# AlexGr5/StereoVision

Measured on AMD Instinct MI355X. Metric: disparity frames/sec + HBM GB/s, 1920x1080 D=128 win=9, 1/2/4/8 GPU, higher is better.
Workload: dtype u8

## Files before the change

### stereovision_amd/csrc/sv_match.hip

```cpp
#include "sv_internal.h"
#include "sv_xcd.h"

#include <algorithm>
#include <cstdlib>
#include <vector>
#include <cstdio>
#include <type_traits>

namespace sv {
namespace {

constexpr int COST_SAD4 = 4;

__host__ __device__ __forceinline__ int seg_width(int lpg, int dpl, int sm = 4) { return (sm * lpg + dpl - 1) / dpl * dpl; }
__host__ __device__ __forceinline__ int wave_cols(int lpg, int dpl, int sm = 4) { return (64 / lpg) * seg_width(lpg, dpl, sm); }
int seg_mult(int kind, int r) {
    static const int sm4 = [] {
        const char* e = std::getenv("SV_SAD4_SEG");
        const int v = e ? std::atoi(e) : 0;
        return v >= 1 && v <= 8 ? v : 0;
    }();
    if (kind != COST_SAD4) return 4;
    if (sm4) return sm4;
    return (2 * r - 2 + 3) / 4 <= 2 ? 4 : 2;
// ... 376 lines not shown
                    h[k][q] = __builtin_amdgcn_sad_hi_u8(L.w[NC + q], rn[sk].w[NC + q], h[k][q]) - m;
                }
                continue;
            }
            uint32_t vn[ROWS];
            ccol<COST, ND, NW>(L, rn[sk], vn);
            if constexpr (RUN) {
                uint32_t vo[ROWS];
                ccol<COST, ND, NW>(LO, ro[sk], vo);
#pragma unroll
                for (int q = 0; q < ROWS; ++q) h[k][q] = shl_add(vn[q] - vo[q], 1 << dbits, h[k][q]);
            } else {
                h[k][0] = (vn[0] << dbits) | mk[k];
            }
        }
#pragma unroll
        for (int q = 0; q < ROWS; ++q) {
            uint32_t b = 0xFFFFFFFFu;
#pragma unroll
            for (int k = 0; k < DPL; ++k) b = min(b, h[k][q]);
            bk[q][u] = b;
        }
        __builtin_amdgcn_sched_barrier(0);
    }
}

template <int LPG, int N>
__device__ __forceinline__ void reduce_batch(uint32_t* v) {
#define SV_ROR_STEP(CTRL)                                                                     \
    _Pragma("unroll") for (int i = 0; i < N; ++i)                                             \
        v[i] = min(v[i], (uint32_t)__builtin_amdgcn_update_dpp(0u, (int)v[i], CTRL, 0xF, 0xF, false));
    SV_ROR_STEP(0x121)
    SV_ROR_STEP(0x122)
    SV_ROR_STEP(0x124)
    SV_ROR_STEP(0x128)
#undef SV_ROR_STEP
    if constexpr (LPG >= 32) {
#pragma unroll
        for (int i = 0; i < N; ++i)
            v[i] = min(v[i], (uint32_t)__builtin_amdgcn_update_dpp(-1, (int)v[i], 0x142, 0xA, 0xF, false));
    }
    if constexpr (LPG == 64) {
#pragma unroll
        for (int i = 0; i < N; ++i)
            v[i] = min(v[i], (uint32_t)__builtin_amdgcn_update_dpp(-1, (int)v[i], 0x143, 0xC, 0xF, false));
    }
}

__device__ __forceinline__ void reduce_scatter16(uint32_t (&v)[16], int l) {
#define SV_RS_STEP(HALF, BIT, CTRL)                                                            \
    {                                                                                          \
        const bool hi = (l & (BIT)) != 0;                                                      \
        _Pragma("unroll") for (int k = 0; k < (HALF); ++k) {                                   \
            const uint32_t send = hi ? v[k] : v[k + (HALF)];                                   \
            const uint32_t keep = hi ? v[k + (HALF)] : v[k];                                   \
            v[k] = min(keep, (uint32_t)__builtin_amdgcn_update_dpp(0u, (int)send, CTRL, 0xF, 0xF, false)); \
        }                                                                                      \
    }
    SV_RS_STEP(8, 8, 0x140)
    SV_RS_STEP(4, 4, 0x141)
    SV_RS_STEP(2, 2, 0x1B)
    SV_RS_STEP(1, 1, 0xB1)
#undef SV_RS_STEP
}

__device__ __forceinline__ void reduce_scatter16_bm(uint32_t (&v)[16], int l) {
#define SV_BM_PAIR(A, B, CTRL, M0, M1)                                                          \
    "v_min_u32_dpp %" #A ", %" #A ", %" #A " " CTRL " row_mask:0xf bank_mask:" M0 "\n\t"      \
    "v_min_u32_dpp %" #A ", %" #B ", %" #B " " CTRL " row_mask:0xf bank_mask:" M1 "\n\t"
    asm volatile("s_nop 1\n\t"
                 SV_BM_PAIR(0, 8, "row_mirror", "0x3", "0xc") SV_BM_PAIR(1, 9, "row_mirror", "0x3", "0xc")
                 SV_BM_PAIR(2, 10, "row_mirror", "0x3", "0xc") SV_BM_PAIR(3, 11, "row_mirror", "0x3", "0xc")
                 SV_BM_PAIR(4, 12, "row_mirror", "0x3", "0xc") SV_BM_PAIR(5, 13, "row_mirror", "0x3", "0xc")
                 SV_BM_PAIR(6, 14, "row_mirror", "0x3", "0xc") SV_BM_PAIR(7, 15, "row_mirror", "0x3", "0xc")
                 : "+v"(v[0]), "+v"(v[1]), "+v"(v[2]), "+v"(v[3]), "+v"(v[4]), "+v"(v[5]), "+v"(v[6]), "+v"(v[7])
                 : "v"(v[8]), "v"(v[9]), "v"(v[10]), "v"(v[11]), "v"(v[12]), "v"(v[13]), "v"(v[14]), "v"(v[15]));
    asm volatile("s_nop 1\n\t"
                 SV_BM_PAIR(0, 4, "row_half_mirror", "0x5", "0xa") SV_BM_PAIR(1, 5, "row_half_mirror", "0x5", "0xa")
                 SV_BM_PAIR(2, 6, "row_half_mirror", "0x5", "0xa") SV_BM_PAIR(3, 7, "row_half_mirror", "0x5", "0xa")
                 : "+v"(v[0]), "+v"(v[1]), "+v"(v[2]), "+v"(v[3])
                 : "v"(v[4]), "v"(v[5]), "v"(v[6]), "v"(v[7]));
#undef SV_BM_PAIR
#define SV_RS_STEP(HALF, BIT, CTRL)                                                            \
    {                                                                                          \
        const bool hi = (l & (BIT)) != 0;                                                      \
        _Pragma("unroll") for (int k = 0; k < (HALF); ++k) {                                   \
            const uint32_t send = hi ? v[k] : v[k + (HALF)];                                   \
            const uint32_t keep = hi ? v[k + (HALF)] : v[k];                                   \
            v[k] = min(keep, (uint32_t)__builtin_amdgcn_update_dpp(0u, (int)send, CTRL, 0xF, 0xF, false)); \
        }                                                                                      \
    }
    SV_RS_STEP(2, 2, 0x1B)
    SV_RS_STEP(1, 1, 0xB1)
#undef SV_RS_STEP
}

__device__ __forceinline__ void reduce_scatter8_bm(uint32_t (&v)[8], int l) {
#define SV_BM_PAIR(A, B, CTRL, M0, M1)                                                          \
    "v_min_u32_dpp %" #A ", %" #A ", %" #A " " CTRL " row_mask:0xf bank_mask:" M0 "\n\t"      \
    "v_min_u32_dpp %" #A ", %" #B ", %" #B " " CTRL " row_mask:0xf bank_mask:" M1 "\n\t"
    asm volatile("s_nop 1\n\t"
                 SV_BM_PAIR(0, 4, "row_mirror", "0x3", "0xc") SV_BM_PAIR(1, 5, "row_mirror", "0x3", "0xc")
                 SV_BM_PAIR(2, 6, "row_mirror", "0x3", "0xc") SV_BM_PAIR(3, 7, "row_mirror", "0x3", "0xc")
                 : "+v"(v[0]), "+v"(v[1]), "+v"(v[2]), "+v"(v[3])
                 : "v"(v[4]), "v"(v[5]), "v"(v[6]), "v"(v[7]));
    asm volatile("s_nop 1\n\t"
                 SV_BM_PAIR(0, 2, "row_half_mirror", "0x5", "0xa") SV_BM_PAIR(1, 3, "row_half_mirror", "0x5", "0xa")
                 : "+v"(v[0]), "+v"(v[1])
                 : "v"(v[2]), "v"(v[3]));
#undef SV_BM_PAIR
    const bool hi = (l & 2) != 0;
    const uint32_t send = hi ? v[0] : v[1];
    const uint32_t keep = hi ? v[1] : v[0];
    v[0] = min(keep, (uint32_t)__builtin_amdgcn_update_dpp(0u, (int)send, 0x1B, 0xF, 0xF, false));
    v[0] = min(v[0], (uint32_t)__builtin_amdgcn_update_dpp(0u, (int)v[0], 0xB1, 0xF, 0xF, false));
}

template <int COST, int ND> struct Occ {
    static constexpr int W = COST == COST_SAD4 ? 2 : (COST == COST_SAD || ND <= 3) ? 3 : 2;
};

template <int COST, int ND, int DPL>
__global__ __launch_bounds__((64 * PackCfg<COST, ND>::WPB), (Occ<COST, ND>::W)) void k_match(MatchParams a) {
    constexpr int NW = PackCfg<COST, ND>::NW;
    constexpr int ROWS = PackCfg<COST, ND>::ROWS;
    extern __shared__ __attribute__((aligned(16))) uint4 smem[];
    if (blockIdx.z) {
        a.L += blockIdx.z * a.fs_in;
        a.R += blockIdx.z * a.fs_in;
        a.out += blockIdx.z * a.fs_out;
        if constexpr (COST == COST_HOG) {
            a.HL += blockIdx.z * a.fs_hist;
            a.HR += blockIdx.z * a.fs_hist;
        }
    }
    const int lane = threadIdx.x & 63;
    const int wid = PackCfg<COST, ND>::WPB == 1 ? 0 : (int)(threadIdx.x >> 6);
    const int LPG = a.lpg;
    const int S = seg_width(LPG, DPL, a.segm);
    const int WC = wave_cols(LPG, DPL, a.segm);
    const int r = a.r;
    const int W2 = 2 * r + 1;
    const int c0 = (DPL - (4 * r + 1) % DPL) % DPL;
    const int NL = WC + 4 * r + DPL + 1;
    const int NRlog = WC + 4 * r + LPG * DPL + DPL;
    const int NRphys = NRlog + (NRlog + c0) / DPL + 1;
    using P = PackCfg<COST, ND>;
    uint4* wbase = reinterpret_cast<uint4*>(reinterpret_cast<char*>(smem) + (size_t)wid * (NL + NRphys) * P::SLOT_BYTES);
    typename P::CT* cbase = reinterpret_cast<typename P::CT*>(wbase + (size_t)(NL + NRphys) * P::QX);
    const PackOut<COST, ND> Lw{wbase, cbase};
    const PackOut<COST, ND> Rw{wbase + (size_t)NL * P::QX, cbase + NL};
    const PackPtr<COST, ND> Lp{Lw.x, Lw.c};
    const PackPtr<COST, ND> Rp{Rw.x, Rw.c};

    const int y = a.row0 + ((int)blockIdx.y * PackCfg<COST, ND>::WPB + wid) * ROWS;
    const int yc = min(y, a.row1 - 1);
    const int xw = a.X0 + (int)blockIdx.x * WC;
    const int cL0 = xw - 3 * r - 1;
    const int cR0 = cL0 - a.minD - (LPG * DPL - 1);

    build_all_packs<COST, ND, DPL>(a, yc, cL0, NL, cR0, NRlog, c0, Lw, Rw, lane);

    if (blockIdx.x == 0) {
        const int16_t inv = (int16_t)((a.minD - 1) * 16);
#pragma unroll
        for (int q = 0; q < ROWS; ++q) {
            if (y + q >= a.row1) break;
            int16_t* orow = a.out + (size_t)(y + q) * a.opitch;
            for (int x = lane; x < a.X0; x += 64) orow[x] = inv;
            for (int x = a.X1 + lane; x < a.W; x += 64) orow[x] = inv;
        }
    }
    __syncthreads();
    if (y >= a.row1) return;

    const int g = lane >> a.lpg_log2;
    const int l = lane & (LPG - 1);
    const int sl = l ^ (((lane >> 4) & 1) << 3);
    const int xs = xw + g * S;
    const int iL0 = g * S + 2 * r + 1;
    const int iR0 = g * S + 2 * r + (LPG - sl) * DPL;
    const uint32_t dmask = (1u << a.dbits) - 1u;
    const int dbits = a.dbits;
    const int j = l - (LPG - 16);

    uint32_t mk[DPL];
    uint32_t h[DPL][ROWS], bk[ROWS][DPL];
#pragma unroll
    for (int k = 0; k < DPL; ++k) {
        const int idx = sl * DPL + k;
        mk[k] = idx < a.D ? (uint32_t)idx : 0xFFFFFFFFu;
#pragma unroll
        for (int q = 0; q < ROWS; ++q) h[k][q] = idx < a.D ? (uint32_t)idx : a.pad_key | (uint32_t)idx;
    }

    for (int t = 0; t < W2; ++t) {
        const Pk<NW> L = ld<COST, ND>(Lp + (iL0 + t));
#pragma unroll
        for (int k = 0; k < DPL; ++k) {
            uint32_t vn[ROWS];
            ccol<COST, ND, NW>(L, ld<COST, ND>(Rp + rslot(iR0 + t - k, c0, DPL)), vn);
            if constexpr (COST == COST_HOG) h[k][0] = (vn[0] << dbits) | mk[k];
            else {
#pragma unroll
                for (int q = 0; q < ROWS; ++q) h[k][q] += vn[q] << dbits;
            }
        }
    }
    {
        const bool emit0 = j == 0 && xs < a.X1;
#pragma unroll
        for (int q = 0; q < ROWS; ++q) {
            uint32_t b = 0xFFFFFFFFu;
#pragma unroll
            for (int k = 0; k < DPL; ++k) b = min(b, h[k][q]);
            if (LPG == 16) reduce_batch<16, 1>(&b);
            else if (LPG == 32) reduce_batch<32, 1>(&b);
            else reduce_batch<64, 1>(&b);
            if (emit0 && y + q < a.row1)
                a.out[(size_t)(y + q) * a.opitch + xs] = (int16_t)(((int)(b & dmask) + a.minD) * 16);
        }
    }

    const int phi = (DPL - W2 % DPL) % DPL;
    const int cut = DPL - phi;
    const int iN = iR0 + W2;
    Pk<NW> rn[DPL], ro[DPL];
#pragma unroll
    for (int s = 1; s < DPL; ++s) {
        rn[s] = ld<COST, ND>(Rp + rslot(iN - (DPL - s), c0, DPL));
        if constexpr (COST != COST_HOG) ro[s] = ld<COST, ND>(Rp + rslot(iR0 - (DPL - s), c0, DPL));
    }
    const PackPtr<COST, ND> rn0 = Rp + rslot(iN, c0, DPL);
    const PackPtr<COST, ND> ro0 = Rp + rslot(iR0, c0, DPL);
    const PackPtr<COST, ND> ln0 = Lp + (iL0 + W2);
    const PackPtr<COST, ND> lo0 = Lp + iL0;
    const int T = (S - 1 + DPL - 1) / DPL * DPL;

    for (int t0 = 0, c = 0; t0 < T; t0 += DPL, ++c) {
        match_chunk<COST, ND, DPL>(cut, dbits, rn0 + c * (DPL + 1), ro0 + c * (DPL + 1), ln0 + t0, lo0 + t0, rn,
                                   ro, h, mk, bk);
        if constexpr (ROWS * DPL == 16 || ROWS * DPL == 32) {
            if (LPG == 16) {
#pragma unroll
                for (int half = 0; half < ROWS * DPL / 16; ++half) {
                    uint32_t v[16];
#pragma unroll
                    for (int i = 0; i < 16; ++i) v[i] = bk[(16 * half + i) / DPL][i % DPL];
                    reduce_scatter16(v, l);
                    const int q = (16 * half) / DPL + l / DPL, e = t0 + l % DPL + 1, x = xs + e;
                    if (e < S && x < a.X1 && y + q < a.row1)
                        a.out[(size_t)(y + q) * a.opitch + x] = (int16_t)(((int)(v[0] & dmask) + a.minD) * 16);
                }
                continue;
            }
        }
        if constexpr (ROWS * DPL == 8) {
            uint32_t v[8];
#pragma unroll
            for (int i = 0; i < 8; ++i) v[i] = bk[i / DPL][i % DPL];
            reduce_scatter8_bm(v, lane & 15);
            uint32_t key = v[0];
            if (LPG >= 32) {
                const auto p = __builtin_amdgcn_permlane16_swap(key, key, false, false);
                key = min(p[0], p[1]);
            }
            if (LPG == 64) {
                const auto p = __builtin_amdgcn_permlane32_swap(key, key, false, false);
                key = min(p[0], p[1]);
            }
            const int i = (l >> 1) & 7, q = i / DPL, e = t0 + i % DPL + 1, x = xs + e;
            if (l < 16 && (l & 1) == 0 && e < S && x < a.X1 && y + q < a.row1)
                a.out[(size_t)(y + q) * a.opitch + x] = (int16_t)(((int)(key & dmask) + a.minD) * 16);
            continue;
        }
        const int e = t0 + j + 1;
        const int x = xs + e;
        const bool emit = j >= 0 && j < DPL && e < S && x < a.X1;
        if (LPG == 16) reduce_batch<16, ROWS * DPL>(&bk[0][0]);
        else if (LPG == 32) reduce_batch<32, ROWS * DPL>(&bk[0][0]);
        else reduce_batch<64, ROWS * DPL>(&bk[0][0]);
#pragma unroll
        for (int q = 0; q < ROWS; ++q) {
            uint32_t v = bk[q][0];
#pragma unroll
            for (int u = 1; u < DPL; ++u) v = (j == u) ? bk[q][u] : v;
            if (emit && y + q < a.row1)
                a.out[(size_t)(y + q) * a.opitch + x] = (int16_t)(((int)(v & dmask) + a.minD) * 16);
        }
    }
}

constexpr int RG_DPL = 4;

typedef unsigned short u16x2 __attribute__((ext_vector_type(2)));
__device__ __forceinline__ uint32_t pk_add16(uint32_t a, uint32_t b) {
    return __builtin_bit_cast(uint32_t, __builtin_bit_cast(u16x2, a) + __builtin_bit_cast(u16x2, b));
}
__device__ __forceinline__ uint32_t pk_sub16(uint32_t a, uint32_t b) {
    return __builtin_bit_cast(uint32_t, __builtin_bit_cast(u16x2, a) - __builtin_bit_cast(u16x2, b));
}


template <int R, int LPGT, bool DEFER, bool KEYS, bool SSD = false>
__global__ __launch_bounds__(64, 2) void k_match_ring(MatchParams a) {
    using P = PackCfg<COST_SAD4, R>;
    constexpr int NW = P::NW, NC = P::NC, W2 = 2 * R + 1;
    constexpr bool PK = R >= 6;
    static_assert(P::SPLIT && (P::CW == 3) == PK, "ring kind expects split packs (20 B for r 2..3, 24 B for r 4..5, 28 B for r 6..7)");
    extern __shared__ __attribute__((aligned(16))) uint4 smem[];
    int bx, by, bz;
    xcd_tile(a.xcd_map != 0, bx, by, bz);
    if (bz) {
        a.L += bz * a.fs_in;
        a.R += bz * a.fs_in;
        a.out += bz * a.fs_out;
        if constexpr (KEYS) a.keys += bz * a.fs_out;
    }
    const int lane = threadIdx.x;
    constexpr int LPG = LPGT;
    const int S = a.segm;
    const int WC = (64 / LPG) * S;
    constexpr bool SADU = PK || R <= 5;
    constexpr int M = SADU ? W2 + 1 : W2;
    constexpr int U = M % 4 == 0 ? M : M % 2 == 0 ? 2 * M : 4 * M;
    constexpr int NCH = U / 4;
    const int Tn = (S + 2 * R + 3) & ~3;
    const int nit = (Tn + U - 1) / U;
    const int e0 = (nit * U - Tn) >> 2;
    const int NL = WC - S + Tn + 1;
    const int NRlog = WC - S + Tn + 4 * LPG;
    constexpr int c0 = 1;
    const int NRphys = NRlog + (NRlog + c0) / RG_DPL + 1;
    uint4* wbase = smem;
    typename P::CT* cbase = reinterpret_cast<typename P::CT*>(wbase + (size_t)(NL + NRphys));
    const PackOut<COST_SAD4, R> Lw{wbase, cbase};
    const PackOut<COST_SAD4, R> Rw{wbase + NL, cbase + NL};
    const PackPtr<COST_SAD4, R> Lp{Lw.x, Lw.c};
    const PackPtr<COST_SAD4, R> Rp{Rw.x, Rw.c};

    const int y = a.row0 + by * 4;
    const int yc = min(y, a.row1 - 1);
    const int xw = a.X0 + bx * WC;
    const int cL0 = xw - R;
    const int cR0 = cL0 - a.minD - (4 * LPG - 1);
    build_ring_packs<R, 3, RG_DPL>(a, yc, cL0, NL, cR0, NRlog, c0, Lw, Rw, lane);

    if (!KEYS && bx == 0) {
        const int16_t inv = (int16_t)((a.minD - 1) * 16);
#pragma unroll
        for (int q = 0; q < 4; ++q) {
            if (y + q >= a.row1) break;
            int16_t* orow = a.out + (size_t)(y + q) * a.opitch;
            for (int x = lane; x < a.X0; x += 64) orow[x] = inv;
            for (int x = a.X1 + lane; x < a.W; x += 64) orow[x] = inv;
        }
    }
    __syncthreads();
    if (y >= a.row1) return;

    const int g = lane / LPG;
    const int l = lane & (LPG - 1);
    const int xs = xw + g * S;
    const int dl = PK ? min(4 * l, a.D - 4) : 4 * l;
    const int iR0 = g * S + 4 * (LPG - 1) - dl + 3;
    constexpr int RQ = PK ? 2 : 4;
    uint32_t h[RG_DPL][RQ], lab[RG_DPL];
#pragma unroll
    for (int k = 0; k < RG_DPL; ++k) {
        const int idx = 4 * l + k;
        const uint32_t base = PK ? 0u : idx < a.D ? (uint32_t)idx : (SSD ? a.pad_key : 0x8000u << 16) | (uint32_t)idx;
        lab[k] = (uint32_t)idx;
#pragma unroll
        for (int q = 0; q < RQ; ++q) h[k][q] = base;
    }
    uint32_t ring[M][RG_DPL][RQ];
#pragma unroll
    for (int s = 0; s < M; ++s)
#pragma unroll
        for (int k = 0; k < RG_DPL; ++k)
#pragma unroll
            for (int q = 0; q < RQ; ++q) ring[s][k][q] = 0u;
    Pk<NW> rn[RG_DPL];
#pragma unroll
    for (int s = 1; s < RG_DPL; ++s) rn[RG_DPL - s] = ld<COST_SAD4, R, true>(Rp + rslot(iR0 - s, c0, RG_DPL));
    PackPtr<COST_SAD4, R> rb = Rp + (rslot(iR0, c0, RG_DPL) - e0 * (RG_DPL + 1));
    PackPtr<COST_SAD4, R> lb = Lp + (g * S - 4 * e0);
    constexpr bool LPF = !(R == 5 && SADU);
    Pk<NW> Lnext = ld<COST_SAD4, R, true>(lb + 4 * e0);
    const int jq = (lane >> 2) & 3, ju = (lane >> 1) & 1;
    constexpr bool join2 = LPG >= 32;
    int pofs = 0;
    if (join2) {
        const auto p = __builtin_amdgcn_permlane16_swap((uint32_t)lane, (uint32_t)lane + 64u, false, false);
        pofs = (max(p[0], p[1]) < 64u) ? 0 : 2;
    }
    const int eb = ju - 2 * R + pofs;
    constexpr int OB = KEYS ? 4 : 2;
    const int ooff = OB * ((y + jq) * a.opitch + xs + eb);
    const auto orsrc = KEYS ? __builtin_amdgcn_make_buffer_rsrc(a.keys, 0, 0x7FFFFFFF, 0x00020000)
                            : __builtin_amdgcn_make_buffer_rsrc(a.out, 0, 0x7FFFFFFF, 0x00020000);
    const int emax = ((l & 1) == 0 && l < (join2 ? 32 : 16) && y + jq < a.row1) ? max(0, min(S, a.X1 - xs)) : 0;

    auto emit_key = [&](uint32_t key, int tt) {
        const int off = (unsigned)(tt + eb) < (unsigned)emax ? ooff + OB * tt : (int)0x80000000u;
        if constexpr (KEYS) __builtin_amdgcn_raw_buffer_store_b32(key, orsrc, off, 0, 0);
        else __builtin_amdgcn_raw_buffer_store_b16(
            (uint16_t)(((int)(key & (SSD ? (1u << a.dbits) - 1u : 0xFFFFu)) + a.minD) * 16), orsrc, off, 0, 0);
    };
    auto join_pairs = [&](uint32_t kA_, uint32_t kB_) {
        auto p = __builtin_amdgcn_permlane16_swap(kA_, kB_, false, false);
        uint32_t key = min(p[0], p[1]);
        if (LPG == 64) {
            p = __builtin_amdgcn_permlane32_swap(key, key, false, false);
            key = min(p[0], p[1]);
        }
        return key;
    };
    auto join_rows = [&](uint32_t key) {
        if (LPG >= 32) {
            const auto p = __builtin_amdgcn_permlane16_swap(key, key, false, false);
            key = min(p[0], p[1]);
        }
        if (LPG == 64) {
            const auto p = __builtin_amdgcn_permlane32_swap(key, key, false, false);
            key = min(p[0], p[1]);
        }
        return key;
    };
    uint32_t dv[8], kA = 0xFFFFFFFFu;
    int tprev = -(1 << 24);
#pragma unroll
    for (int i = 0; i < 8; ++i) dv[i] = 0xFFFFFFFFu;

    for (int it = 0, t0 = -4 * e0; it < nit; ++it) {
#pragma unroll
        for (int ch = 0; ch < NCH; ++ch, t0 += 4) {
            if (t0 < 0) continue;
            uint32_t bk[4][2];
#pragma unroll
            for (int u = 0; u < 4; ++u) {
                const int slot = (4 * ch + u) % M, oslot = (4 * ch + u + 1) % M;
                rn[u] = ld<COST_SAD4, R, true>(rb + (ch * (RG_DPL + 1) + u));
                const Pk<NW> Lc = LPF ? Lnext : ld<COST_SAD4, R, true>(lb + (4 * ch + u));
                if constexpr (LPF) Lnext = ld<COST_SAD4, R, true>(lb + (4 * ch + u + 1));
                uint32_t sqL[4];
                if constexpr (SSD) {
                    uint32_t sc = 0u;
#pragma unroll
                    for (int i = 0; i < NC; ++i) sc = __builtin_amdgcn_udot4(Lc.w[i], Lc.w[i], sc, false);
#pragma unroll
                    for (int q = 0; q < 4; ++q)
                        sqL[q] = __builtin_amdgcn_udot4(Lc.w[NC + q], Lc.w[NC + q], sc, false) << a.dbits;
                }
                if constexpr (!SADU) {
#pragma unroll
                    for (int k = 0; k < RG_DPL; ++k)
#pragma unroll
                        for (int q = 0; q < RQ; ++q)
                            h[k][q] = PK ? pk_sub16(h[k][q], ring[slot][k][q]) : h[k][q] - ring[slot][k][q];
                }
#pragma unroll
                for (int kk = 0; kk < RG_DPL; ++kk) {
                    const int k = RG_DPL - 1 - kk;
                    const Pk<NW>& Rk = rn[(u - k) & 3];
                    if constexpr (PK) {
                        uint32_t cn = 0u;
#pragma unroll
                        for (int i = 0; i < NC; ++i) cn = __builtin_amdgcn_sad_u8(Lc.w[i], Rk.w[i], cn);
                        cn |= cn << 16;
#pragma unroll
                        for (int j = 0; j < 2; ++j) {
                            const uint32_t c = __builtin_amdgcn_sad_hi_u8(
                                Lc.w[NC + 2 * j + 1], Rk.w[NC + 2 * j + 1],
                                __builtin_amdgcn_sad_u8(Lc.w[NC + 2 * j], Rk.w[NC + 2 * j], cn));
                            if constexpr (SADU) sad_u32_acc(h[k][j], ring[oslot][k][j], c);
                            else h[k][j] = pk_add16(h[k][j], c);
                            ring[slot][k][j] = c;
                        }
                    } else if constexpr (SSD) {
                        uint32_t cn = 0u, sr = 0u;
#pragma unroll
                        for (int i = 0; i < NC; ++i) {
                            cn = __builtin_amdgcn_udot4(Lc.w[i], Rk.w[i], cn, false);
                            sr = __builtin_amdgcn_udot4(Rk.w[i], Rk.w[i], sr, false);
                        }
#pragma unroll
                        for (int q = 0; q < 4; ++q) {
                            const uint32_t lr = __builtin_amdgcn_udot4(Lc.w[NC + q], Rk.w[NC + q], cn, false);
                            const uint32_t rr = __builtin_amdgcn_udot4(Rk.w[NC + q], Rk.w[NC + q], sr, false);
                            const uint32_t t = (rr << a.dbits) + sqL[q];
                            const uint32_t c = (uint32_t)__mul24((int)lr, -(2 << a.dbits)) + t;
                            sad_u32_acc(h[k][q], ring[oslot][k][q], c);
                            ring[slot][k][q] = c;
                        }
                    } else {
                        uint32_t cn = 0u;
#pragma unroll
                        for (int i = 0; i < NC; ++i) cn = __builtin_amdgcn_sad_hi_u8(Lc.w[i], Rk.w[i], cn);
#pragma unroll
                        for (int q = 0; q < 4; ++q) {
                            const uint32_t c = __builtin_amdgcn_sad_hi_u8(Lc.w[NC + q], Rk.w[NC + q], cn);
                            if constexpr (SADU) sad_u32_acc(h[k][q], ring[oslot][k][q], c);
                            else h[k][q] += c;
                            ring[slot][k][q] = c;
                        }
                    }
                }
#pragma unroll
                for (int q = 0; q < 4; ++q) {
                    uint32_t kq[RG_DPL];
#pragma unroll
                    for (int k = 0; k < RG_DPL; ++k)
                        kq[k] = !PK ? h[k][q] : (q & 1) ? (h[k][q >> 1] & 0xFFFF0000u) | lab[k] : (h[k][q >> 1] << 16) | lab[k];
                    bk[q][u & 1] = min(min(kq[0], kq[1]), min(kq[2], kq[3]));
                }
                __builtin_amdgcn_sched_barrier(0);
                if (DEFER && u == 3) {
#pragma unroll
                    for (int i = 0; i < 8; ++i) dv[i] = bk[i >> 1][i & 1];
                } else if (DEFER && u == 1) {
                    uint32_t v[8];
#pragma unroll
                    for (int i = 0; i < 8; ++i) v[i] = bk[i >> 1][i & 1];
                    reduce_scatter8_bm(v, lane & 15);
                    reduce_scatter8_bm(dv, lane & 15);
                    if (join2) {
                        emit_key(join_pairs(kA, dv[0]), tprev);
                        kA = v[0];
                    } else {
                        emit_key(join_rows(dv[0]), tprev + 2);
                        emit_key(join_rows(v[0]), t0);
                    }
                    tprev = t0;
                } else if (u & 1) {
                    uint32_t v[8];
#pragma unroll
                    for (int i = 0; i < 8; ++i) v[i] = bk[i >> 1][i & 1];
                    reduce_scatter8_bm(v, lane & 15);
                    if (join2) {
                        if (u == 1) kA = v[0];
                        else emit_key(join_pairs(kA, v[0]), t0);
                    } else {
                        emit_key(join_rows(v[0]), t0 + u - 1);
                    }
                }
            }
        }
        rb = rb + NCH * (RG_DPL + 1);
        lb = lb + U;
    }
    if (DEFER) {
        reduce_scatter8_bm(dv, lane & 15);
        if (join2) emit_key(join_pairs(kA, dv[0]), tprev);
        else emit_key(join_rows(dv[0]), tprev + 2);
    }
}

__global__ void k_fill_i16(int16_t* out, int opitch, int H, int W, int16_t v) {
    const int x = blockIdx.x * blockDim.x + threadIdx.x;
    const int y = blockIdx.y;
    if (x < W && y < H) out[(size_t)y * opitch + x] = v;
}

template <int COST, int ND, int DPL>
int launch_one(const MatchParams& a, size_t lds, hipStream_t s) {
    auto fn = k_match<COST, ND, DPL>;
    if (lds > 65536) {
        hipError_t e = hipFuncSetAttribute((const void*)fn, hipFuncAttributeMaxDynamicSharedMemorySize, (int)lds);
        if (e != hipSuccess) return (int)e;
    }
    const int wc = wave_cols(a.lpg, DPL, a.segm);
    const int rows_per_block = PackCfg<COST, ND>::WPB * PackCfg<COST, ND>::ROWS;
    dim3 grid((a.X1 - a.X0 + wc - 1) / wc, (a.row1 - a.row0 + rows_per_block - 1) / rows_per_block,
              a.nf > 1 ? a.nf : 1);
    hipLaunchKernelGGL(fn, grid, dim3(64 * PackCfg<COST, ND>::WPB), lds, s, a);
    return (int)hipGetLastError();
}

template <int COST, int ND>
int launch_dpl(const MatchParams& a, const MatchPlan& p, size_t lds, hipStream_t s) {
    switch (p.dpl) {
        case 4: return launch_one<COST, ND, 4>(a, lds, s);
        case 6: return launch_one<COST, ND, 6>(a, lds, s);
        case 8: return launch_one<COST, ND, 8>(a, lds, s);
    }
    return (int)hipErrorInvalidValue;
}

template <int COST>
int launch_nd(const MatchParams& a, const MatchPlan& p, size_t lds, hipStream_t s) {
    if constexpr (COST == COST_HOG) {
        return launch_dpl<COST, 5>(a, p, lds, s);
    } else if constexpr (COST == COST_SAD4) {
        switch (p.ndw) {
            case 2: return launch_dpl<COST, 2>(a, p, lds, s);
            case 3: return launch_dpl<COST, 3>(a, p, lds, s);
            case 4: return launch_dpl<COST, 4>(a, p, lds, s);
            case 5: return launch_dpl<COST, 5>(a, p, lds, s);
            case 6: return launch_dpl<COST, 6>(a, p, lds, s);
            case 7: return launch_dpl<COST, 7>(a, p, lds, s);
        }
        return (int)hipErrorInvalidValue;
    } else {
        switch (p.ndw) {
            case 1: return launch_dpl<COST, 1>(a, p, lds, s);
            case 2: return launch_dpl<COST, 2>(a, p, lds, s);
            case 3: return launch_dpl<COST, 3>(a, p, lds, s);
            case 4: return launch_dpl<COST, 4>(a, p, lds, s);
        }
        return (int)hipErrorInvalidValue;
    }
}

int kind_of(int cost, int win) {
    if (cost == COST_SAD && win >= 5) return COST_SAD4;
    return cost;
}

bool ring_kind(int cost, int win, int num_disp) {
    static const bool on = [] {
        const char* e = std::getenv("SV_RING");
        return !(e && e[0] == '0');
    }();
    return on && kind_of(cost, win) == COST_SAD4 && win >= 5 && num_disp <= 256 &&
           (win <= 11 || (win <= 15 && num_disp % 4 == 0));
}
int ring_lpg(int num_disp) { return num_disp <= 64 ? 16 : num_disp <= 128 ? 32 : 64; }
size_t ring_lds_bytes(int lpg, int seg, int r);
int ring_seg(int lpg, int r, int band, long long blocks) {
    static const int env = [] {
        const char* e = std::getenv("SV_RING_SEG");
        const int v = e ? std::atoi(e) : 0;
        return v >= 8 && v <= 1024 && v % 4 == 0 ? v : 0;
    }();
    (void)blocks;
    if (env) return env;
    const int G = 64 / lpg;
    int best = 8;
    long long best_cost = -1;
    for (int S = 8; S <= 1024; S += 4) {
        if (S > 8 && ring_lds_bytes(lpg, S, r) > 20 * 1024) break;
        const long long cost = (long long)((band + G * S - 1) / (G * S)) * ((S + 2 * r + 3) & ~3);
        if (best_cost < 0 || cost <= best_cost) { best = S; best_cost = cost; }
    }
    return best;
}
size_t ring_lds_bytes(int lpg, int seg, int r) {
    const int wc = (64 / lpg) * seg;
    const int tn = (seg + 2 * r + 3) & ~3;
    const int nl = wc - seg + tn + 1, nr = wc - seg + tn + 4 * lpg;
    const int nrp = nr + (nr + 1) / RG_DPL + 1;
    return (size_t)(nl + nrp) * (r <= 3 ? 20 : r <= 5 ? 24 : 28);
}

template <int R, int LPG, bool KEYS, bool SSD>
int launch_ring_rl(const MatchParams& a, size_t lds, hipStream_t s) {
    static const bool defer = [] {
        const char* e = std::getenv("SV_RING_DEFER");
        return !(e && e[0] == '0');
    }();
    void (*fn)(MatchParams);
    if constexpr (SSD) fn = k_match_ring<R, LPG, R != 5, false, true>;
    else if constexpr (KEYS) fn = k_match_ring<R, LPG, R != 5, true>;
    else fn = (defer && R != 5) ? k_match_ring<R, LPG, R != 5, false> : k_match_ring<R, LPG, false, false>;
    if (lds > 65536) {
        hipError_t e = hipFuncSetAttribute((const void*)fn, hipFuncAttributeMaxDynamicSharedMemorySize, (int)lds);
        if (e != hipSuccess) return (int)e;
    }
    const int wc = (64 / a.lpg) * a.segm;
    dim3 grid((a.X1 - a.X0 + wc - 1) / wc, (a.row1 - a.row0 + 3) / 4, a.nf > 1 ? a.nf : 1);
    static const bool xcd = [] {
        const char* e = std::getenv("SV_XCD_MAP");
        return !(e && e[0] == '0');
    }();
    MatchParams b = a;
    b.xcd_map = xcd ? 1 : 0;
    hipLaunchKernelGGL(fn, grid, dim3(64), lds, s, b);
    return (int)hipGetLastError();
}
template <int R, bool KEYS, bool SSD = false>
int launch_ring_r(const MatchParams& a, size_t lds, hipStream_t s) {
    switch (a.lpg) {
        case 16: return launch_ring_rl<R, 16, KEYS, SSD>(a, lds, s);
        case 32: return launch_ring_rl<R, 32, KEYS, SSD>(a, lds, s);
        case 64: return launch_ring_rl<R, 64, KEYS, SSD>(a, lds, s);
    }
    return (int)hipErrorInvalidValue;
}

template <bool KEYS, bool SSD = false>
int launch_ring(const MatchParams& a0, hipStream_t s) {
    MatchParams a = a0;
    a.lpg = ring_lpg(a.D);
    a.lpg_log2 = a.lpg == 16 ? 4 : a.lpg == 32 ? 5 : 6;
    a.dbits = SSD ? a.lpg_log2 + 2 : 16;
    if (SSD) a.pad_key = (uint32_t)((max_cost(a.win, COST_SSD) + 1) << a.dbits);
    a.segm = ring_seg(a.lpg, a.r, a.X1 - a.X0, (long long)((a.row1 - a.row0 + 3) / 4) * (a.nf > 1 ? a.nf : 1));
    const size_t lds = ring_lds_bytes(a.lpg, a.segm, a.r);
    if (lds > 160 * 1024) return (int)hipErrorInvalidValue;
    if constexpr (SSD) {
        switch (a.r) {
            case 2: return launch_ring_r<2, false, true>(a, lds, s);
            case 3: return launch_ring_r<3, false, true>(a, lds, s);
            case 4: return launch_ring_r<4, false, true>(a, lds, s);
        }
        return (int)hipErrorInvalidValue;
    } else {
        switch (a.r) {
            case 2: return launch_ring_r<2, KEYS>(a, lds, s);
            case 3: return launch_ring_r<3, KEYS>(a, lds, s);
            case 4: return launch_ring_r<4, KEYS>(a, lds, s);
            case 5: return launch_ring_r<5, KEYS>(a, lds, s);
            case 6: return launch_ring_r<6, KEYS>(a, lds, s);
            case 7: return launch_ring_r<7, KEYS>(a, lds, s);
        }
        return (int)hipErrorInvalidValue;
    }
}

__device__ __forceinline__ int16_t merge_px(uint32_t ka, uint32_t kb, int x, int X0, int X1, int minD) {
    const uint32_t k = min(ka, kb + 256u);
    return (int16_t)(x >= X0 && x < X1 ? ((int)(k & 0xFFFFu) + minD) * 16 : (minD - 1) * 16);
}
__global__ __launch_bounds__(256) void k_merge_ring_keys(const uint32_t* __restrict__ ka,
                                                         const uint32_t* __restrict__ kb, int16_t* __restrict__ out,
                                                         int opitch, long long fs_out, int row0, int W, int X0, int X1,
                                                         int minD, int vec) {
    const int x = 4 * (int)(blockIdx.x * 256 + threadIdx.x);
    if (x >= W) return;
    const size_t i = (size_t)blockIdx.z * fs_out + (size_t)(row0 + (int)blockIdx.y) * opitch + x;
    if (vec && x + 4 <= W) {
        const uint4 a = *reinterpret_cast<const uint4*>(ka + i);
        const uint4 b = *reinterpret_cast<const uint4*>(kb + i);
        const uint32_t lo = (uint16_t)merge_px(a.x, b.x, x, X0, X1, minD) |
                            ((uint32_t)(uint16_t)merge_px(a.y, b.y, x + 1, X0, X1, minD) << 16);
        const uint32_t hi = (uint16_t)merge_px(a.z, b.z, x + 2, X0, X1, minD) |
                            ((uint32_t)(uint16_t)merge_px(a.w, b.w, x + 3, X0, X1, minD) << 16);
        *reinterpret_cast<uint2*>(out + i) = make_uint2(lo, hi);
        return;
    }
    for (int q = 0; q < 4 && x + q < W; ++q) out[i + q] = merge_px(ka[i + q], kb[i + q], x + q, X0, X1, minD);
}


}

bool ring_ssd(int cost, int win, int num_disp) {
    if (cost != COST_SSD || win < 5 || win > 9 || num_disp < 1 || num_disp > 256) return false;
    if (!ring_kind(COST_SAD, win, num_disp)) return false;
    const int lpg = ring_lpg(num_disp), dbits = (lpg == 16 ? 4 : lpg == 32 ? 5 : 6) + 2;
    const uint64_t cmax = max_cost(win, COST_SSD);
    const uint64_t top = num_disp < 4 * lpg ? (2 * cmax + 2) << dbits : (cmax << dbits) + (uint64_t)(4 * lpg);
    return top < (1ull << 32);
}
bool ring_split(int cost, int win, int num_disp) {
    return num_disp > 256 && num_disp <= 512 && ring_kind(cost, win, 256) && ring_kind(cost, win, num_disp - 256);
}
long long ring_split_elems(int nf, long long fs_out, int row1, int opitch) {
    return ((long long)(nf > 1 ? nf - 1 : 0) * fs_out + (long long)(row1 + 3) * opitch + 64 + 3) & ~3LL;
}

uint64_t max_cost(int win, int cost) {
    return cost == COST_SAD ? (uint64_t)win * win * 255
         : cost == COST_SSD ? (uint64_t)win * win * 255 * 255
                            : (uint64_t)9 * win * win * 255;
}

int plan_match(int num_disp, int win, int cost, MatchPlan* plan) {
    static const int menu[][2] = {{4, 16}, {6, 16}, {8, 16}, {6, 32}, {8, 32}, {6, 64}, {8, 64}};
    if (num_disp <= 0 || win < 1 || (win & 1) == 0 || win > 15) return -22;
    if (cost != COST_SAD && cost != COST_SSD && cost != COST_HOG) return -22;
    int i = 0;
    for (; i < 7; ++i)
        if (menu[i][0] * menu[i][1] >= num_disp) break;
    if (i == 7) return -22;
    plan->dpl = menu[i][0];
    plan->lpg = menu[i][1];
    const int kind = kind_of(cost, win);
    plan->ndw = kind == COST_HOG ? 5 : kind == COST_SAD4 ? win / 2
              : (win + 3) / 4;
    int n = plan->dpl * plan->lpg - 1, bits = 0;
    while (n > 0) { ++bits; n >>= 1; }
    plan->dbits = bits < 1 ? 1 : bits;
    if (hi_keys(kind, win / 2)) plan->dbits = 16;
    const uint64_t cmax = max_cost(win, cost);
    const bool over = (cmax << plan->dbits) >= (1ull << 32) ||
                      (num_disp < plan->dpl * plan->lpg && cost != COST_HOG &&
                       ((2 * cmax + 2) << plan->dbits) >= (1ull << 32));
    plan->mfma_only = 0;
    if (over) {
        if (!ssd_mfma(cost, win, num_disp)) return -34;
        plan->mfma_only = 1;
    }
    return 0;
}

size_t match_lds_bytes(const MatchPlan& p, int r, int cost) {
    const int kind = kind_of(cost, 2 * r + 1);
    const int nw = kind == COST_SAD ? p.ndw : kind == COST_SSD ? p.ndw + 1
                 : kind == COST_SAD4 ? (2 * p.ndw - 2 + 3) / 4 + 4 : 5;
    const int wpb = kind == COST_SAD4 ? 1 : 4;
    const bool split = (kind == COST_SAD4 && nw - 4 <= 3) || kind == COST_HOG || (kind == COST_SSD && nw == 5);
    const int cw = kind == COST_SAD4 && nw - 4 == 3 ? 3 : kind == COST_SAD4 && nw - 4 == 1 ? 1 : 2;
    const int Q = (nw + 3) / 4;
    const int c0 = (p.dpl - (4 * r + 1) % p.dpl) % p.dpl;
    const int wc = wave_cols(p.lpg, p.dpl, seg_mult(kind, r));
    const int NL = wc + 4 * r + p.dpl + 1;
    const int NRlog = wc + 4 * r + p.lpg * p.dpl + p.dpl;
    const int NRphys = NRlog + (NRlog + c0) / p.dpl + 1;
    return (size_t)wpb * (NL + NRphys) * (split ? 16 + 4 * cw : Q * 16);
}

int launch_fill_i16(int16_t* out, int opitch, int H, int W, int16_t v, hipStream_t s) {
    if (H <= 0 || W <= 0) return 0;
    hipLaunchKernelGGL(k_fill_i16, dim3((W + 255) / 256, H), dim3(256), 0, s, out, opitch, H, W, v);
    return (int)hipGetLastError();
}

int launch_match(const MatchParams& a, const MatchPlan& p, int cost, hipStream_t s) {
    if (a.row1 <= a.row0) return 0;
    if (a.X1 <= a.X0) {
        for (int z = 0; z < (a.nf > 1 ? a.nf : 1); ++z) {
            int e = launch_fill_i16(a.out + z * a.fs_out + (size_t)a.row0 * a.opitch, a.opitch,
                                    a.row1 - a.row0, a.W, (int16_t)((a.minD - 1) * 16), s);
            if (e) return e;
        }
        return 0;
    }
    const bool ring_fits = 2LL * ((long long)(a.row1 + 3) * a.opitch + a.W + 64) < 0x7FFFFFFFLL;
    if (ring_kind(cost, a.win, a.D) && ring_fits) return launch_ring<false>(a, s);
    if (ssd_mfma_fits(a, cost)) return launch_ssd_mfma(a, s);
    if (p.mfma_only) return (int)hipErrorInvalidValue;
    if (ring_ssd(cost, a.win, a.D) && ring_fits) return launch_ring<false, true>(a, s);
    if (ring_split(cost, a.win, a.D) && a.keys) {
        if (4LL * ((long long)(a.row1 + 3) * a.opitch + a.W + 64) >= 0x7FFFFFFFLL) return (int)hipErrorInvalidValue;
        MatchParams pa = a, pb = a;
        pa.D = 256;
        pb.minD = a.minD + 256;
        pb.D = a.D - 256;
        pb.keys = a.keys + a.keys_stride;
        int e = launch_ring<true>(pa, s);
        if (!e) e = launch_ring<true>(pb, s);
        if (e) return e;
        const int nf = a.nf > 1 ? a.nf : 1;
        const long long fso = nf > 1 ? a.fs_out : 0LL;
        const int vec = (a.opitch % 4 == 0 && fso % 4 == 0 && a.keys_stride % 4 == 0 &&
                         ((uintptr_t)a.out & 7) == 0 && ((uintptr_t)a.keys & 15) == 0) ? 1 : 0;
        hipLaunchKernelGGL(k_merge_ring_keys, dim3((a.W + 1023) / 1024, a.row1 - a.row0, nf), dim3(256), 0, s, pa.keys,
                           pb.keys, a.out, a.opitch, fso, a.row0, a.W, a.X0, a.X1, a.minD, vec);
        return (int)hipGetLastError();
    }
    const size_t lds = match_lds_bytes(p, a.r, cost);
    if (lds > 160 * 1024) return (int)hipErrorInvalidValue;
    MatchParams b = a;
    b.segm = seg_mult(kind_of(cost, a.win), a.r);
    switch (kind_of(cost, a.win)) {
        case COST_SAD: return launch_nd<COST_SAD>(b, p, lds, s);
        case COST_SAD4: return launch_nd<COST_SAD4>(b, p, lds, s);
        case COST_SSD: return launch_nd<COST_SSD>(b, p, lds, s);
        case COST_HOG: return launch_nd<COST_HOG>(b, p, lds, s);
    }
    return (int)hipErrorInvalidValue;
}

}
```

Baseline: 30700.

## Fold ring-kernel disparity minima through LDS scratch instead of cross-lane permlane reductions

Adds an LDSMIN variant of the ring matcher, enabled by default for lpg=32 and r=4 (D=128, win=9) SAD output. Each pair of disparity steps writes the eight per-lane best keys into a 2 KB LDS scratch with ds_write_addtid. On the following step each lane reads back two 16-byte vectors and folds them with min plus two DPP swizzles, which replaces the deferred reduce_scatter and permlane joins. The output-lane mapping and store predicate change to match. The scratch shrinks the LDS left for segments and adds LDS traffic and wavefront fences inside the inner loop. There is also an env-gated occupancy print.

```diff
diff --git a/stereovision_amd/csrc/sv_match.hip b/stereovision_amd/csrc/sv_match.hip
--- a/stereovision_amd/csrc/sv_match.hip
+++ b/stereovision_amd/csrc/sv_match.hip
@@ -702,10 +702,14 @@
 }
 
 
-template <int R, int LPGT, bool DEFER, bool KEYS, bool SSD = false>
+typedef uint32_t lds_u32x4 __attribute__((ext_vector_type(4), may_alias));
+constexpr int RING_SCRATCH_BYTES = 8 * 64 * 4;
+
+template <int R, int LPGT, bool DEFER, bool KEYS, bool SSD = false, bool LDSMIN = false>
 __global__ __launch_bounds__(64, 2) void k_match_ring(MatchParams a) {
     using P = PackCfg<COST_SAD4, R>;
     constexpr int NW = P::NW, NC = P::NC, W2 = 2 * R + 1;
+    static_assert(!LDSMIN || (LPGT == 32 && R <= 5), "the LDS fold is laid out for two 32-lane groups of 32-bit keys");
     constexpr bool PK = R >= 6;
     static_assert(P::SPLIT && (P::CW == 3) == PK, "ring kind expects split packs (20 B for r 2..3, 24 B for r 4..5, 28 B for r 6..7)");
     extern __shared__ __attribute__((aligned(16))) uint4 smem[];
@@ -732,7 +736,7 @@
     const int NRlog = WC - S + Tn + 4 * LPG;
     constexpr int c0 = 1;
     const int NRphys = NRlog + (NRlog + c0) / RG_DPL + 1;
-    uint4* wbase = smem;
+    uint4* wbase = smem + (LDSMIN ? RING_SCRATCH_BYTES / 16 : 0);
     typename P::CT* cbase = reinterpret_cast<typename P::CT*>(wbase + (size_t)(NL + NRphys));
     const PackOut<COST_SAD4, R> Lw{wbase, cbase};
     const PackOut<COST_SAD4, R> Rw{wbase + NL, cbase + NL};
@@ -791,16 +795,20 @@
     const int jq = (lane >> 2) & 3, ju = (lane >> 1) & 1;
     constexpr bool join2 = LPG >= 32;
     int pofs = 0;
-    if (join2) {
+    if (join2 && !LDSMIN) {
         const auto p = __builtin_amdgcn_permlane16_swap((uint32_t)lane, (uint32_t)lane + 64u, false, false);
         pofs = (max(p[0], p[1]) < 64u) ? 0 : 2;
     }
-    const int eb = ju - 2 * R + pofs;
+    const int eq = LDSMIN ? lane >> 4 : jq;
+    const int exs = LDSMIN ? xw + ((lane >> 2) & 1) * S : xs;
+    const int eb = (LDSMIN ? ((lane >> 3) & 1) + 2 * (lane & 1) : ju + pofs) - 2 * R;
     constexpr int OB = KEYS ? 4 : 2;
-    const int ooff = OB * ((y + jq) * a.opitch + xs + eb);
+    const int ooff = OB * ((y + eq) * a.opitch + exs + eb);
     const auto orsrc = KEYS ? __builtin_amdgcn_make_buffer_rsrc(a.keys, 0, 0x7FFFFFFF, 0x00020000)
                             : __builtin_amdgcn_make_buffer_rsrc(a.out, 0, 0x7FFFFFFF, 0x00020000);
-    const int emax = ((l & 1) == 0 && l < (join2 ? 32 : 16) && y + jq < a.row1) ? max(0, min(S, a.X1 - xs)) : 0;
+    const int emax = (LDSMIN ? (lane & 2) == 0 && y + eq < a.row1
+                             : (l & 1) == 0 && l < (join2 ? 32 : 16) && y + jq < a.row1)
+                         ? max(0, min(S, a.X1 - exs)) : 0;
 
     auto emit_key = [&](uint32_t key, int tt) {
         const int off = (unsigned)(tt + eb) < (unsigned)emax ? ooff + OB * tt : (int)0x80000000u;
@@ -832,6 +840,20 @@
     int tprev = -(1 << 24);
 #pragma unroll
     for (int i = 0; i < 8; ++i) dv[i] = 0xFFFFFFFFu;
+    [[maybe_unused]] uint32_t* const scr = reinterpret_cast<uint32_t*>(smem);
+    [[maybe_unused]] const uint32_t scr_m0 = __builtin_amdgcn_readfirstlane(
+        (uint32_t)(uintptr_t)(__attribute__((address_space(3))) uint32_t*)scr);
+    [[maybe_unused]] const lds_u32x4* const sra = reinterpret_cast<const lds_u32x4*>(scr + 8 * lane + 4 * ((lane >> 3) & 1));
+    [[maybe_unused]] const lds_u32x4* const srb = reinterpret_cast<const lds_u32x4*>(scr + 8 * lane + 4 * (1 - ((lane >> 3) & 1)));
+    auto lds_fold = [&](const lds_u32x4& p, const lds_u32x4& s) {
+        uint32_t m = min(min(p.x, p.y), p.z);
+        m = min(min(m, p.w), s.x);
+        m = min(min(m, s.y), s.z);
+        m = min(m, s.w);
+        m = min(m, (uint32_t)__builtin_amdgcn_update_dpp(0u, (int)m, 0xB1, 0xF, 0xF, false));
+        return min(m, (uint32_t)__builtin_amdgcn_update_dpp(0u, (int)m, 0x4E, 0xF, 0xF, false));
+    };
+    [[maybe_unused]] const bool pairB = (lane & 1) != 0;
 
     for (int it = 0, t0 = -4 * e0; it < nit; ++it) {
 #pragma unroll
@@ -844,6 +866,10 @@
                 rn[u] = ld<COST_SAD4, R, true>(rb + (ch * (RG_DPL + 1) + u));
                 const Pk<NW> Lc = LPF ? Lnext : ld<COST_SAD4, R, true>(lb + (4 * ch + u));
                 if constexpr (LPF) Lnext = ld<COST_SAD4, R, true>(lb + (4 * ch + u + 1));
+                lds_u32x4 fa{}, fb{};
+                if constexpr (LDSMIN) {
+                    if ((u & 1) == 0) { fa = *sra; fb = *srb; }
+                }
                 uint32_t sqL[4];
                 if constexpr (SSD) {
                     uint32_t sc = 0u;
@@ -915,7 +941,36 @@
                         kq[k] = !PK ? h[k][q] : (q & 1) ? (h[k][q >> 1] & 0xFFFF0000u) | lab[k] : (h[k][q >> 1] << 16) | lab[k];
                     bk[q][u & 1] = min(min(kq[0], kq[1]), min(kq[2], kq[3]));
                 }
+                if constexpr (LDSMIN) {
+                    if (u == 2) {
+                        kA = lds_fold(fa, fb);
+                    } else if (u == 0) {
+                        const uint32_t kB = lds_fold(fa, fb);
+                        emit_key(pairB ? kB : kA, tprev);
+                        tprev = t0;
+                    }
+                }
                 __builtin_amdgcn_sched_barrier(0);
+                if constexpr (LDSMIN) {
+                    if (u & 1) {
+                        asm volatile("s_mov_b32 m0, %8\n\t"
+                                     "s_nop 0\n\t"
+                                     "ds_write_addtid_b32 %0\n\t"
+                                     "ds_write_addtid_b32 %1 offset:256\n\t"
+                                     "ds_write_addtid_b32 %2 offset:512\n\t"
+                                     "ds_write_addtid_b32 %3 offset:768\n\t"
+                                     "ds_write_addtid_b32 %4 offset:1024\n\t"
+                                     "ds_write_addtid_b32 %5 offset:1280\n\t"
+                                     "ds_write_addtid_b32 %6 offset:1536\n\t"
+                                     "ds_write_addtid_b32 %7 offset:1792\n\t"
+                                     :
+                                     : "v"(bk[0][0]), "v"(bk[0][1]), "v"(bk[1][0]), "v"(bk[1][1]), "v"(bk[2][0]),
+                                       "v"(bk[2][1]), "v"(bk[3][0]), "v"(bk[3][1]), "s"(scr_m0)
+                                     : "memory", "m0");
+                        __builtin_amdgcn_fence(__ATOMIC_SEQ_CST, "wavefront");
+                    }
+                    continue;
+                }
                 if (DEFER && u == 3) {
 #pragma unroll
                     for (int i = 0; i < 8; ++i) dv[i] = bk[i >> 1][i & 1];
@@ -950,7 +1005,10 @@
         rb = rb + NCH * (RG_DPL + 1);
         lb = lb + U;
     }
-    if (DEFER) {
+    if constexpr (LDSMIN) {
+        const uint32_t kB = lds_fold(*sra, *srb);
+        emit_key(pairB ? kB : kA, tprev);
+    } else if (DEFER) {
         reduce_scatter8_bm(dv, lane & 15);
         if (join2) emit_key(join_pairs(kA, dv[0]), tprev);
         else emit_key(join_rows(dv[0]), tprev + 2);
@@ -1027,8 +1085,15 @@
            (win <= 11 || (win <= 15 && num_disp % 4 == 0));
 }
 int ring_lpg(int num_disp) { return num_disp <= 64 ? 16 : num_disp <= 128 ? 32 : 64; }
-size_t ring_lds_bytes(int lpg, int seg, int r);
-int ring_seg(int lpg, int r, int band, long long blocks) {
+bool ring_ldsmin(int lpg, int r, bool keys, bool ssd) {
+    static const bool on = [] {
+        const char* e = std::getenv("SV_RING_LDSMIN");
+        return !(e && e[0] == '0');
+    }();
+    return on && lpg == 32 && r == 4 && !keys && !ssd;
+}
+size_t ring_lds_bytes(int lpg, int seg, int r, bool ldsmin);
+int ring_seg(int lpg, int r, int band, long long blocks, bool ldsmin) {
     static const int env = [] {
         const char* e = std::getenv("SV_RING_SEG");
         const int v = e ? std::atoi(e) : 0;
@@ -1040,18 +1105,18 @@
     int best = 8;
     long long best_cost = -1;
     for (int S = 8; S <= 1024; S += 4) {
-        if (S > 8 && ring_lds_bytes(lpg, S, r) > 20 * 1024) break;
+        if (S > 8 && ring_lds_bytes(lpg, S, r, ldsmin) > 20 * 1024) break;
         const long long cost = (long long)((band + G * S - 1) / (G * S)) * ((S + 2 * r + 3) & ~3);
         if (best_cost < 0 || cost <= best_cost) { best = S; best_cost = cost; }
     }
     return best;
 }
-size_t ring_lds_bytes(int lpg, int seg, int r) {
+size_t ring_lds_bytes(int lpg, int seg, int r, bool ldsmin) {
     const int wc = (64 / lpg) * seg;
     const int tn = (seg + 2 * r + 3) & ~3;
     const int nl = wc - seg + tn + 1, nr = wc - seg + tn + 4 * lpg;
     const int nrp = nr + (nr + 1) / RG_DPL + 1;
-    return (size_t)(nl + nrp) * (r <= 3 ? 20 : r <= 5 ? 24 : 28);
+    return (size_t)(nl + nrp) * (r <= 3 ? 20 : r <= 5 ? 24 : 28) + (ldsmin ? RING_SCRATCH_BYTES : 0);
 }
 
 template <int R, int LPG, bool KEYS, bool SSD>
@@ -1064,12 +1129,25 @@
     if constexpr (SSD) fn = k_match_ring<R, LPG, R != 5, false, true>;
     else if constexpr (KEYS) fn = k_match_ring<R, LPG, R != 5, true>;
     else fn = (defer && R != 5) ? k_match_ring<R, LPG, R != 5, false> : k_match_ring<R, LPG, false, false>;
+    if constexpr (R == 4 && LPG == 32 && !KEYS && !SSD) {
+        if (ring_ldsmin(LPG, R, KEYS, SSD)) fn = k_match_ring<R, LPG, false, false, false, true>;
+    }
     if (lds > 65536) {
         hipError_t e = hipFuncSetAttribute((const void*)fn, hipFuncAttributeMaxDynamicSharedMemorySize, (int)lds);
         if (e != hipSuccess) return (int)e;
     }
     const int wc = (64 / a.lpg) * a.segm;
     dim3 grid((a.X1 - a.X0 + wc - 1) / wc, (a.row1 - a.row0 + 3) / 4, a.nf > 1 ? a.nf : 1);
+    static const bool occ = [] {
+        const char* e = std::getenv("SV_RING_OCC");
+        return e && e[0] == '1';
+    }();
+    if (occ) {
+        int nb = -1;
+        (void)hipOccupancyMaxActiveBlocksPerMultiprocessor(&nb, (const void*)fn, 64, lds);
+        std::fprintf(stderr, "k_match_ring r=%d lpg=%d ldsmin=%d seg=%d lds=%zu B: %d waves/CU\n", R, LPG,
+                     (int)ring_ldsmin(LPG, R, KEYS, SSD), a.segm, lds, nb);
+    }
     static const bool xcd = [] {
         const char* e = std::getenv("SV_XCD_MAP");
         return !(e && e[0] == '0');
@@ -1096,8 +1174,9 @@
     a.lpg_log2 = a.lpg == 16 ? 4 : a.lpg == 32 ? 5 : 6;
     a.dbits = SSD ? a.lpg_log2 + 2 : 16;
     if (SSD) a.pad_key = (uint32_t)((max_cost(a.win, COST_SSD) + 1) << a.dbits);
-    a.segm = ring_seg(a.lpg, a.r, a.X1 - a.X0, (long long)((a.row1 - a.row0 + 3) / 4) * (a.nf > 1 ? a.nf : 1));
-    const size_t lds = ring_lds_bytes(a.lpg, a.segm, a.r);
+    const bool ldsmin = ring_ldsmin(a.lpg, a.r, KEYS, SSD);
+    a.segm = ring_seg(a.lpg, a.r, a.X1 - a.X0, (long long)((a.row1 - a.row0 + 3) / 4) * (a.nf > 1 ? a.nf : 1), ldsmin);
+    const size_t lds = ring_lds_bytes(a.lpg, a.segm, a.r, ldsmin);
     if (lds > 160 * 1024) return (int)hipErrorInvalidValue;
     if constexpr (SSD) {
         switch (a.r) {
```

Result: faster. 31100 (median of 6 runs) (+1.3%).
